# honglu2875/hironaka

Hardware: AMD Instinct MI355X
Metric: env-steps/sec at dim=3, max_pts=20, batch=65536; 1/2/4/8 GPUs (higher is better)
Workload: dtype f32

## Files before the change

hironaka_amd/csrc/hk_duo_kernel.h:

```cpp
#pragma once

#include "hk_fast_kernel.h"
#include "hk_lds_dma.h"

namespace hk {

constexpr int kDuoGames = kWave / 2;

#ifndef HK_DUO_LEGS
#define HK_DUO_LEGS 3
#endif
#ifdef HK_DUO_PROBE
constexpr int kDuoProbeRow = 48, kDuoProbeWaves = 4096;
static __device__ int32_t duo_probe_rows[kDuoProbeWaves * kDuoProbeRow];
#define HK_DUO_PROBE_PARAM , int32_t* probe = nullptr
#define HK_DUO_PROBE_ARG(p) , p
#else
#define HK_DUO_PROBE_PARAM
#define HK_DUO_PROBE_ARG(p)
#endif
constexpr bool kDuoLegDma = (HK_DUO_LEGS & 1) != 0, kDuoLegScan = (HK_DUO_LEGS & 2) != 0;

__device__ __forceinline__ int duo_other_i(int v) { return qperm_i<0xB1>(v); }
__device__ __forceinline__ float duo_other(float v) { return __int_as_float(duo_other_i(__float_as_int(v))); }

__device__ __forceinline__ uint64_t duo_ballot(bool p) { return __builtin_amdgcn_ballot_w64(p); }

template <int M, int D>
struct DuoGeom {
  using G = FastGeom<M, D>;
  static constexpr int CH = (G::C + 1) / 2;
  static constexpr int QH = (kDuoGames * G::Q + kWave - 1) / kWave;
  static constexpr bool kLean = CH * D <= 30;
};

template <int M, int D>
struct DuoSlabRegs {
  typename VecOf<FastGeom<M, D>::W>::type v[DuoGeom<M, D>::QH];
};

template <int M, int D, bool CONTIG>
__device__ __forceinline__ void duo_slab_issue_impl(DuoSlabRegs<M, D>& r, const float* base, int64_t in_stride,
                                                    int ngames, int lane) {
  using G = FastGeom<M, D>;
  using V = typename VecOf<G::W>::type;
  const int total = ngames * G::Q;
#pragma unroll
  for (int it = 0; it < DuoGeom<M, D>::QH; ++it) {
    int q = lane + it * kWave;
    q = q < total ? q : total - 1;
    r.v[it] = *reinterpret_cast<const V*>(base + slab_chunk_global<M, D, CONTIG>(q, in_stride));
  }
}

template <int M, int D>
__device__ __forceinline__ void duo_slab_issue(DuoSlabRegs<M, D>& r, const float* in, int64_t in_stride, int64_t g0,
                                               int ngames, int lane) {
  const float* base = in + g0 * in_stride;
  if (in_stride == FastGeom<M, D>::N) duo_slab_issue_impl<M, D, true>(r, base, in_stride, ngames, lane);
  else duo_slab_issue_impl<M, D, false>(r, base, in_stride, ngames, lane);
}

template <int M, int D>
__device__ __forceinline__ void duo_slab_commit(DuoSlabRegs<M, D>& r, float* lds, int ngames, int lane) {
  using G = FastGeom<M, D>;
  using V = typename VecOf<G::W>::type;
  const int total = ngames * G::Q;
#pragma unroll
  for (int it = 0; it < DuoGeom<M, D>::QH; ++it) asm volatile("" : "+v"(r.v[it]));
#pragma unroll
  for (int it = 0; it < DuoGeom<M, D>::QH; ++it) {
    const int q = lane + it * kWave;
    if (q < total) *reinterpret_cast<V*>(lds + slab_chunk_lds<M, D>(q)) = r.v[it];
  }
}

template <int M, int D>
struct DuoDma {
  using G = FastGeom<M, D>;
  static constexpr bool kShape = kDuoLegDma && G::W == 4 && G::S == G::N;
};

template <int M, int D>
__device__ __forceinline__ void duo_slab_dma(const float* base, float* image, int ngames, int lane) {
  using G = FastGeom<M, D>;
  constexpr int FULL = kDuoGames * G::Q;
  constexpr int QH = DuoGeom<M, D>::QH;
  constexpr int kImm = kDmaImm;
  static_assert(DuoDma<M, D>::kShape, "the image is the slab");
  const float* src = base + (unsigned)lane * 4;
  const unsigned total = (unsigned)ngames * G::Q;
  if (ngames == kDuoGames) {
    unrolled_while<0, QH>([&](auto ic) {
      constexpr int it = decltype(ic)::value;
      if ((it + 1) * kWave <= FULL || lane < FULL - it * kWave)
        lds_dma<16, (it * kWave * 16) % kImm>(src + (it * kWave * 16) / kImm * (kImm / 4),
                                             image + (it * kWave * 16) / kImm * (kImm / 4));
      return true;
    });
  } else {
    unrolled_while<0, QH>([&](auto ic) {
      constexpr int it = decltype(ic)::value;
      if ((unsigned)lane + it * kWave < total)
        lds_dma<16, (it * kWave * 16) % kImm>(src + (it * kWave * 16) / kImm * (kImm / 4),
                                             image + (it * kWave * 16) / kImm * (kImm / 4));
      return true;
    });
  }
}

constexpr int kStorePlain = 0, kStoreNT = 1, kStoreWT = 2;

template <int M, int D, bool CONTIG, int kBatch, int ST = kStorePlain>
__device__ __forceinline__ void duo_store_slab_impl(const float* lds, float* base, int64_t out_stride, int ngames,
                                                    int lane HK_DUO_PROBE_PARAM) {
  using G = FastGeom<M, D>;
  using V = typename VecOf<G::W>::type;
  constexpr int QH = DuoGeom<M, D>::QH;
  constexpr bool kWT = ST == kStoreWT && CONTIG && G::W == 4;
  const int total = ngames * G::Q;
#pragma unroll
  for (int i0 = 0; i0 < QH; i0 += kBatch) {
    V v[kBatch];
#pragma unroll
    for (int u = 0; u < kBatch; ++u) {
      int q = lane + (i0 + u) * kWave;
      q = q < kDuoGames * G::Q ? q : kDuoGames * G::Q - 1;
      v[u] = *reinterpret_cast<const V*>(lds + slab_chunk_lds<M, D>(q));
    }
#pragma unroll
    for (int u = 0; u < kBatch; ++u) asm volatile("" : "+v"(v[u]));
#ifdef HK_DUO_PROBE
    if (probe && lane == 0) probe[0] = (int32_t)wall_clock64();
#endif
    if constexpr (kWT) {
      typedef unsigned int vu4 __attribute__((ext_vector_type(4)));
      const uint64_t b = (uint64_t)base;
      const uint32_t blo = __builtin_amdgcn_readfirstlane((uint32_t)b), bhi = __builtin_amdgcn_readfirstlane((uint32_t)(b >> 32));
      const int bytes = __builtin_amdgcn_readfirstlane(total * G::W * (int)sizeof(float));
      const auto rsrc = __builtin_amdgcn_make_buffer_rsrc((void*)(((uint64_t)bhi << 32) | blo), 0, bytes, 0x00020000);
#pragma unroll
      for (int u = 0; u < kBatch; ++u) {
        const int q = lane + (i0 + u) * kWave;
        if (i0 + u < QH && q < total)
          __builtin_amdgcn_raw_buffer_store_b128(__builtin_bit_cast(vu4, v[u]), rsrc, q * G::W * (int)sizeof(float), 0,
                                                 16);
      }
    } else {
#pragma unroll
      for (int u = 0; u < kBatch; ++u) {
        const int q = lane + (i0 + u) * kWave;
        if (i0 + u < QH && q < total) {
          V* dst = reinterpret_cast<V*>(base + slab_chunk_global<M, D, CONTIG>(q, out_stride));
          if constexpr (ST != kStorePlain) __builtin_nontemporal_store(v[u], dst);
          else *dst = v[u];
        }
      }
    }
  }
}

template <int M, int D, int kBatch = DuoGeom<M, D>::QH, int ST = kStorePlain>
__device__ inline void duo_store_slab(const float* lds, float* out, int64_t out_stride, int64_t g0, int ngames,
                                      int lane HK_DUO_PROBE_PARAM) {
  float* base = out + g0 * out_stride;
  if (out_stride == FastGeom<M, D>::N) duo_store_slab_impl<M, D, true, kBatch, ST>(lds, base, out_stride, ngames, lane HK_DUO_PROBE_ARG(probe));
  else duo_store_slab_impl<M, D, false, kBatch, ST>(lds, base, out_stride, ngames, lane HK_DUO_PROBE_ARG(probe));
#ifdef HK_DUO_PROBE
  if (probe && lane == 0) probe[1] = (int32_t)wall_clock64();
#endif
}

struct DuoLadder {
  static constexpr int next_bucket(int nb) { return nb < 6 ? nb + 1 : nb + 2; }
};

template <int M, int CH, int D, int SB = CH>
__device__ __forceinline__ void duo_gather_slots(float (&q)[CH * D], const float* mine, uint32_t mask, int smax, int h) {
  mask = h ? (mask & (mask - 1)) : mask;
  unrolled_while<0, SB>([&](auto sc) {
    constexpr int s = decltype(sc)::value;
    if (s >= smax) return false;
    const bool has = mask != 0;
    const float* row = mine + (has ? mask_first(mask) : 0) * D;
    mask &= mask - 1;
    mask &= mask - 1;
#pragma unroll
    for (int k = 0; k < D; ++k) {
      const float v = row[k];
      q[s * D + k] = has ? v : INFINITY;
    }
    return true;
  });
}

template <int CH, int D, int NB, int SB = NB>
__device__ __forceinline__ void duo_gather_level(float (&q)[CH * D], const float* mine, const float* hole, uint32_t mask,
                                                 int h) {
  mask = h ? (mask & (mask - 1)) : mask;
  const float* row[NB];
#pragma unroll
  for (int s = 0; s < NB; ++s) {
    row[s] = mask != 0 ? mine + mask_first(mask) * D : hole;
    mask &= mask - 1;
    mask &= mask - 1;
  }
#pragma unroll
  for (int s = 0; s < NB; ++s)
#pragma unroll
    for (int k = 0; k < D; ++k) q[s * D + k] = row[s][k];
#pragma unroll
  for (int e = NB * D; e < SB * D; ++e) q[e] = INFINITY;
}

template <int M, int CH, int D, bool LEVELS, int SB = CH>
__device__ __forceinline__ void duo_gather(float (&q)[CH * D], const float* mine, const float* hole, uint32_t mask,
                                           int smax, int h) {
  if constexpr (LEVELS) {
    StagesFor<DuoLadder, SB>::run(smax, [&](auto nb) {
      duo_gather_level<CH, D, decltype(nb)::value, SB>(q, mine, hole, mask, h);
      return 0;
    });
  } else {
    duo_gather_slots<M, CH, D, SB>(q, mine, mask, smax, h);
  }
}

template <int CH, int D, int NB>
__device__ __forceinline__ uint32_t duo_scatter_level(const float (&q)[CH * D], float* mine, uint32_t mask, int h) {
  mask = h ? (mask & (mask - 1)) : mask;
  uint32_t alive = 0;
#pragma unroll
  for (int s = 0; s < NB; ++s) {
    if (mask != 0 && q[s * D] < INFINITY) {
      const int slot = mask_first(mask);
      alive |= 1u << slot;
      float* row = mine + slot * D;
#pragma unroll
      for (int k = 0; k < D; ++k) row[k] = q[s * D + k];
    }
    mask &= mask - 1;
    mask &= mask - 1;
  }
  return alive;
}

template <int M, int CH, int D, int SB = CH>
__device__ __forceinline__ uint32_t duo_scatter(const float (&q)[CH * D], float* mine, uint32_t mask, int smax, int h) {
  mask = h ? (mask & (mask - 1)) : mask;
  uint32_t alive = 0;
  unrolled_while<0, SB>([&](auto sc) {
    constexpr int s = decltype(sc)::value;
    if (s >= smax) return false;
    if (mask != 0 && q[s * D] < INFINITY) {
      const int slot = mask_first(mask);
      alive |= 1u << slot;
      float* row = mine + slot * D;
#pragma unroll
      for (int k = 0; k < D; ++k) row[k] = q[s * D + k];
    }
    mask &= mask - 1;
    mask &= mask - 1;
    return true;
  });
  return lanes_or<2>(alive);
}

template <int D>
__device__ __forceinline__ void duo_pad_rows(float* mine, uint32_t dead, float pad, int h) {
  dead = h ? (dead & (dead - 1)) : dead;
  while (dead != 0) {
    float* row = mine + mask_first(dead) * D;
#pragma unroll
    for (int k = 0; k < D; ++k) row[k] = pad;
    dead &= dead - 1;
    dead &= dead - 1;
  }
}

template <int M, int D>
__device__ __forceinline__ void duo_scan_half(const float* mine, float fill, int h, uint32_t& live, bool& ok) {
  static_assert(M <= 32, "the game's mask is one word");
  constexpr int C = (M + 1) / 2;
  const int i0 = h * C;
  const float* base = mine + i0 * D;
  uint32_t mask = 0;
  const uint32_t fill_bits = __float_as_uint(fill);
  uint32_t off = 0;
  bool okb = true;
#pragma unroll
  for (int r = 0; r < C; ++r) {
    const bool valid = (M % 2 == 0) || r + 1 < C || h == 0;
    uint32_t hi = __float_as_uint(base[r * D]), lo = hi;
#pragma unroll
    for (int k = 1; k < D; ++k) {
      const uint32_t u = __float_as_uint(base[r * D + k]);
      hi = u > hi ? u : hi;
      lo = u < lo ? u : lo;
    }
    const bool ge = hi < 0x7F800000u;
    if constexpr (DuoGeom<M, D>::kLean && kDuoLegScan) {
      const uint32_t differs = (hi ^ fill_bits) | (lo ^ fill_bits);
      off |= (ge || !valid) ? 0u : differs;
    } else {
      const bool fl = (lo == fill_bits) && (hi == fill_bits);
      okb &= (ge | fl | !valid);
    }
    mask |= (ge && valid) ? (1u << r) : 0u;
  }
  ok = (DuoGeom<M, D>::kLean && kDuoLegScan) ? off == 0u : okb;
  mask <<= i0;
  live = lanes_or<2>(mask);
}

template <bool DPP>
__device__ __forceinline__ int duo_wave_max(int v, int hi) {
  if constexpr (!DPP) return wave_max(v, hi);
  auto mx = [](int a, int b) { return a > b ? a : b; };
  v = mx(v, __builtin_amdgcn_update_dpp(0, v, 0x111, 0xF, 0xF, true));
  v = mx(v, __builtin_amdgcn_update_dpp(0, v, 0x112, 0xF, 0xF, true));
  v = mx(v, __builtin_amdgcn_update_dpp(0, v, 0x114, 0xF, 0xF, true));
  v = mx(v, __builtin_amdgcn_update_dpp(0, v, 0x118, 0xF, 0xF, true));
  v = mx(v, __builtin_amdgcn_update_dpp(0, v, 0x142, 0xA, 0xF, false));
  v = mx(v, __builtin_amdgcn_update_dpp(0, v, 0x143, 0xC, 0xF, false));
  return __builtin_amdgcn_readlane(v, kWave - 1);
}

template <int CH, int D, int NB>
__device__ __forceinline__ void d_newton(float (&q)[CH * D], int h) {
  float acc[NB], oth[NB];
#pragma unroll
  for (int i = 0; i + 1 < NB; ++i) {
#pragma unroll
    for (int j = i + 1; j < NB; ++j) {
      float t, u;
      diff_extrema<D>(&q[i * D], &q[j * D], t, u);
      const float vi = (t > 0.0f) ? -u : 1.0f;
      acc[j] = (i == 0) ? t : hk_fmin(acc[j], t);
      acc[i] = (i == 0 && j == 1) ? vi : hk_fmin(acc[i], vi);
    }
    __builtin_amdgcn_sched_barrier(0);
  }
  const bool late = h != 0;
#pragma unroll
  for (int b = 0; b < NB; ++b) {
    float o[D];
#pragma unroll
    for (int k = 0; k < D; ++k) o[k] = duo_other(q[b * D + k]);
    {
      float t, u;
      diff_extrema<D>(&q[b * D], o, t, u);
      const float va = (t > 0.0f || late) ? -u : 1.0f;
      acc[b] = (NB == 1) ? va : hk_fmin(acc[b], va);
      oth[b] = (u < 0.0f || !late) ? t : 1.0f;
    }
#pragma unroll
    for (int a = 0; a < b; ++a) {
      float t, u;
      diff_extrema<D>(&q[a * D], o, t, u);
      oth[b] = hk_fmin(oth[b], t);
      acc[a] = hk_fmin(acc[a], (t > 0.0f) ? -u : 1.0f);
    }
    __builtin_amdgcn_sched_barrier(0);
  }
#pragma unroll
  for (int r = 0; r < NB; ++r) {
    const bool r0 = acc[r] <= 0.0f, r1 = duo_other(oth[r]) <= 0.0f;
    const bool removed = r0 || r1;
#pragma unroll
    for (int k = 0; k < D; ++k) q[r * D + k] = removed ? INFINITY : q[r * D + k];
  }
}

template <int CH, int D, int NB>
__device__ __forceinline__ void d_shift_words(float (&q)[CH * D], uint32_t cmask, int axis, int np, unsigned flags) {
  bool apply = true;
  if (flags & HK_FLAG_AXIS_NOOP_IF_INVALID) apply = axis >= 0 && ((cmask >> axis) & 1u);
  if ((flags & HK_FLAG_IGNORE_ENDED) && np < 2) apply = false;
  const uint32_t onehot = apply ? 1u << (axis & 31) : 0u;
  uint32_t isax[D], in[D];
#pragma unroll
  for (int k = 0; k < D; ++k) {
    isax[k] = (uint32_t)((int32_t)(onehot << (31 - k)) >> 31);
    in[k] = (uint32_t)((int32_t)(cmask << (31 - k)) >> 31);
    asm volatile("" : "+v"(isax[k]), "+v"(in[k]));
  }
#pragma unroll
  for (int r = 0; r < NB; ++r) {
    float s = __uint_as_float(__float_as_uint(q[r * D]) & in[0]);
#pragma unroll
    for (int k = 1; k < D; ++k) s = s + __uint_as_float(__float_as_uint(q[r * D + k]) & in[k]);
#pragma unroll
    for (int k = 0; k < D; ++k)
      q[r * D + k] = __uint_as_float((__float_as_uint(s) & isax[k]) | (__float_as_uint(q[r * D + k]) & ~isax[k]));
  }
}

template <int CH, int D, int NB, bool BIN = false, bool WORDS = false>
__device__ __forceinline__ int d_stages(float (&q)[CH * D], const float (&c)[D], int axis, int np, int h,
                                        unsigned flags, unsigned stages, uint32_t cmask = 0) {
  static_assert(!WORDS || BIN, "the subset as bits");
  if (stages & HK_STAGE_SHIFT) {
    if constexpr (WORDS) d_shift_words<CH, D, NB>(q, cmask, axis, np, flags);
    else if constexpr (BIN) b_shift_mask<CH, D, NB>(q, cmask, axis, np, flags);
    else b_shift<CH, D, NB>(q, c, axis, np, flags);
  }
  if (stages & HK_STAGE_REPOSITION) reposition<2, CH, D, NB, BIN>(q, flags);
  if (stages & HK_STAGE_NEWTON) d_newton<CH, D, NB>(q, h);
  if (stages & HK_STAGE_RESCALE) rescale<2, CH, D, NB>(q, flags);
  return live_rows<2, CH, D, NB>(q);
}

template <int CH, int D, int NB, bool BIN = false>
struct DuoStagesFor {
  static constexpr int kNext = DuoLadder::next_bucket(NB);
  static __device__ __forceinline__ int run(float (&q)[CH * D], int smax, const float (&c)[D], int axis, int np,
                                            int h, unsigned flags, unsigned stages, uint32_t cmask = 0) {
    if constexpr (NB >= CH) {
      return d_stages<CH, D, CH, BIN>(q, c, axis, np, h, flags, stages, cmask);
    } else {
      if (smax <= NB) return d_stages<CH, D, NB, BIN>(q, c, axis, np, h, flags, stages, cmask);
      return DuoStagesFor<CH, D, kNext, BIN>::run(q, smax, c, axis, np, h, flags, stages, cmask);
    }
  }
};

template <int CH, int D>
__device__ __forceinline__ void duo_ranks_first(const float (&q)[CH * D], int smax, int (&rank)[CH]) {
#pragma unroll
  for (int s = 0; s < CH; ++s) rank[s] = 0;
  unrolled_while<0, CH>([&](auto bc) {
    constexpr int b = decltype(bc)::value;
    if (b >= smax) return false;
    float o[D];
#pragma unroll
    for (int k = 0; k < D; ++k) o[k] = duo_other(q[b * D + k]);
    const bool live_o = o[0] < INFINITY, live_b = q[b * D] < INFINITY;
    unrolled_while<0, CH>([&](auto ac) {
      constexpr int a = decltype(ac)::value;
      if (a >= smax) return false;
      rank[a] += (live_o && key_gt<D, kKeyFirst>(o, &q[a * D])) ? 1 : 0;
      if (a != b) rank[a] += (live_b && key_gt<D, kKeyFirst>(&q[b * D], &q[a * D])) ? 1 : 0;
      return true;
    });
    return true;
  });
}

template <int CH, int D>
__device__ __forceinline__ void duo_scatter_ranked(const float (&q)[CH * D], float* mine, const int (&rank)[CH], int smax) {
  unrolled_while<0, CH>([&](auto sc) {
    constexpr int s = decltype(sc)::value;
    if (s >= smax) return false;
    if (q[s * D] < INFINITY) {
      float* row = mine + rank[s] * D;
#pragma unroll
      for (int k = 0; k < D; ++k) row[k] = q[s * D + k];
    }
    return true;
  });
}

struct DuoPolicyCache {
  U4 r;
  uint32_t pair = 0xFFFFFFFFu;
};

__device__ inline void duo_policy_words(uint64_t gg, uint32_t step, uint64_t seed, DuoPolicyCache& cache, int h,
                                        uint32_t& host_word, uint32_t& agent_word) {
  const uint32_t block = step >> 2, pair = block >> 1;
  if (cache.pair != pair) {
    cache.r = philox4x32((uint32_t)gg, (uint32_t)(gg >> 32), (pair << 1) | (uint32_t)h, kStreamPolicy, seed);
    cache.pair = pair;
  }
  const uint32_t mine = u4_word(cache.r, step & 3u);
  const bool own = (int)(block & 1u) == h;
  uint32_t theirs = (uint32_t)duo_other_i((int)mine);
  asm volatile("" : "+v"(theirs));
  const uint32_t w = own ? mine : theirs;
  host_word = w & 0xFFFF0000u;
  agent_word = w << 16;
}

constexpr int kDuoZeilDpp = 6;

template <int CH, int D, int NB>
__device__ __forceinline__ int duo_zeillinger(const float (&q)[CH * D], int h, float* mine, int smax) {
  constexpr bool KEEP = NB <= kDuoZeilDpp;
  ZeilBest<D> best;
#pragma unroll
  for (int k = 0; k < D; ++k) best.bd[k] = 0.0f;
  if constexpr (KEEP) {
    float p[NB * D];
#pragma unroll
    for (int e = 0; e < NB * D; ++e) p[e] = duo_other(q[e]);
#pragma unroll
    for (int a = 0; a < NB; ++a) {
#pragma unroll
      for (int b = a + 1; b < NB; ++b)
        zeil_pair_cmp<D, true, false>(best, &q[a * D], &q[b * D], true, (128 * a + 2 * b) + 65 * h);
#pragma unroll
      for (int b = a; b < NB; ++b)
        zeil_pair_cmp<D, true>(best, &q[a * D], &p[b * D], (b > a) | (h == 0), (128 * a + 2 * b + 1) + 63 * h);
      if constexpr (NB > 3) __builtin_amdgcn_sched_barrier(0);
    }
  } else {
    __syncthreads();
#pragma unroll
    for (int s = 0; s < NB; ++s)
#pragma unroll
      for (int k = 0; k < D; ++k) mine[(2 * s + h) * D + k] = q[s * D + k];
    __syncthreads();
    const int n = 2 * smax;
    ZeilBest<D> second;
#pragma nounroll
    for (int i = h; i + 1 < n; i += 2) {
      float pi[D];
#pragma unroll
      for (int k = 0; k < D; ++k) pi[k] = mine[i * D + k];
#pragma nounroll
      for (int j = i + 1; j < n; j += 2) {
        float pj[D], pk[D];
        const int j2 = (j + 1 < n) ? j + 1 : j;
#pragma unroll
        for (int k = 0; k < D; ++k) {
          pj[k] = mine[j * D + k];
          pk[k] = mine[j2 * D + k];
        }
        zeil_pair2<D>(best, second, pi, pj, 64 * i + j, pi, pk, 64 * i + j + 1);
      }
    }
    zeil_merge<D, false>(best, second);
  }
  {
    ZeilBest<D> o;
    o.hi = (uint32_t)duo_other_i((int)best.hi);
    o.lo = (uint32_t)duo_other_i((int)best.lo);
    if constexpr (KEEP) {
#pragma unroll
      for (int k = 0; k < D; ++k) o.bd[k] = duo_other(best.bd[k]);
    }
    zeil_merge<D, KEEP>(best, o);
  }
  const bool have = best.have();
  if constexpr (!KEEP) {
    const int i = have ? (int)((best.lo & 0xFFFFu) >> 6) : 0, j = have ? (int)(best.lo & 63u) : 0;
#pragma unroll
    for (int k = 0; k < D; ++k) best.bd[k] = mine[i * D + k] - mine[j * D + k];
    __syncthreads();
  }
  int lo = 0, hi = 0;
  float vlo = best.bd[0], vhi = best.bd[0];
#pragma unroll
  for (int k = 1; k < D; ++k) {
    if (best.bd[k] < vlo) { vlo = best.bd[k]; lo = k; }
    if (best.bd[k] > vhi) { vhi = best.bd[k]; hi = k; }
  }
  if (!have || lo == hi) return 0;
  return encode_mask((1u << lo) | (1u << hi));
}

constexpr int kDuoPreBlocks = 6;

template <int D>
__device__ __forceinline__ void duo_policy_fill(uint8_t* act, uint64_t gg, uint32_t wb0, int nb, uint64_t seed,
                                                int host_policy, int agent_policy, int gi, int h) {
  static_assert(D <= 5 && D <= kPolicyShortDim, "an action travels as a byte; four steps per Philox block");
  auto put = [&](const U4& r, int b) {
    int cls, axis;
    uint32_t mask;
#pragma unroll
    for (int k = 0; k < 4; ++k) {
      const uint32_t w = u4_word(r, k);
      policy_from_words<D>(w & 0xFFFF0000u, w << 16, host_policy, agent_policy, cls, axis, mask, 0);
      act[(4 * b + k) * kDuoGames + gi] = (uint8_t)(mask | ((uint32_t)axis << 5));
    }
  };
#pragma nounroll
  for (int i = 0; i < kDuoPreBlocks; i += 4) {
    if (i >= nb) break;
    const int b0 = i + h, b1 = b0 + 2;
    if (i + 2 < nb) {
      const U4 r0 = philox4x32((uint32_t)gg, (uint32_t)(gg >> 32), wb0 + (uint32_t)b0, kStreamPolicy, seed);
      const U4 r1 = philox4x32((uint32_t)gg, (uint32_t)(gg >> 32), wb0 + (uint32_t)b1, kStreamPolicy, seed);
      put(r0, b0);
      if (b1 < kDuoPreBlocks) put(r1, b1);
    } else {
      const U4 r0 = philox4x32((uint32_t)gg, (uint32_t)(gg >> 32), wb0 + (uint32_t)b0, kStreamPolicy, seed);
      if (b0 < kDuoPreBlocks) put(r0, b0);
    }
  }
}

template <int M, int D, int MODE, int HOT = kHotNone, bool ACTS = false, bool ZEIL = false>
__global__ __launch_bounds__(kWave, 2) void duo_kernel(const float* in0, int64_t in_stride0, int batch0,
                                                       const Params prm) {
  static_assert(!ACTS || MODE == kModeRollout, "the small records ride on the plain rollout");
  static_assert(!ZEIL || (MODE == kModeRollout && HOT == kHotNone && !ACTS), "Zeillinger's host: plain rollouts");
  constexpr bool kRec = MODE == kModeRolloutRec;
  constexpr bool kRoll = MODE == kModeRollout || kRec;
  constexpr bool kPartialPublish = MODE == kModeRollout && !ZEIL && DuoGeom<M, D>::kLean;
  constexpr bool kLevelDeal = MODE == kModeRollout && DuoGeom<M, D>::kLean;
  using G = FastGeom<M, D>;
  constexpr int CH = DuoGeom<M, D>::CH;
  static_assert(M <= 32, "the live mask of a game travels as 32 bits");
  __shared__ __align__(16) float lds[kDuoGames * G::S];
  __shared__ float cbuf[kDuoGames * D];
  __shared__ float hole_row[D];
  __shared__ __align__(16) uint8_t pol[(MODE == kModeRollout) ? (4 * kDuoPreBlocks + 1) * kDuoGames : 16];
  const int lane = threadIdx.x;
  const int h = lane & 1, gi = lane >> 1;
  const int64_t g0 = (int64_t)blockIdx.x * kDuoGames;
  const int64_t left = (int64_t)batch0 - g0;
  const int ngames = (int)(left < kDuoGames ? left : kDuoGames);
  const bool active = gi < ngames;
  const bool leader = active && h == 0;
  const int64_t g = g0 + gi;
#ifdef HK_DUO_PROBE
  __shared__ int32_t probe_buf[32];
  if (lane < 32) probe_buf[lane] = 0;
  const long long probe_t0 = wall_clock64();
  long long probe_t1 = 0, probe_t2 = 0;
  int probe_steps = 0, probe_smax = 0;
#endif
  const bool has_ids = kRoll && prm.game_ids != nullptr;
  uint32_t raw_id = 0;
  DuoSlabRegs<M, D> slab;
  uint64_t gg;
  bool dma = false;
  if constexpr (DuoDma<M, D>::kShape) {
    if (has_ids) {
      if (active) raw_id = (uint32_t)prm.game_ids[g];
      __builtin_amdgcn_sched_barrier(0);
      duo_slab_issue<M, D>(slab, in0, in_stride0, g0, ngames, lane);
      __builtin_amdgcn_sched_barrier(0);
      asm volatile("" : "+v"(raw_id));
      gg = prm.game_offset + (uint64_t)raw_id;
    } else {
      dma = in_stride0 == G::N && ((uintptr_t)in0 & 15u) == 0;
      if (dma) duo_slab_dma<M, D>(in0 + g0 * G::N, lds, ngames, lane);
      else duo_slab_issue<M, D>(slab, in0, in_stride0, g0, ngames, lane);
      __builtin_amdgcn_sched_barrier(0);
      gg = prm.game_offset + (uint64_t)g;
    }
  } else {
    if (has_ids && active) raw_id = (uint32_t)prm.game_ids[g];
    __builtin_amdgcn_sched_barrier(0);
    duo_slab_issue<M, D>(slab, in0, in_stride0, g0, ngames, lane);
    __builtin_amdgcn_sched_barrier(0);
    gg = prm.game_offset + (has_ids ? (uint64_t)raw_id : (uint64_t)g);
  }
  uint32_t pol_b0 = prm.step_offset >> 2;
  const uint32_t pol_last = (prm.steps > 0) ? (prm.step_offset + (uint32_t)prm.steps - 1u) >> 2 : pol_b0;
  if constexpr (MODE == kModeRollout && !ZEIL) {
    const uint32_t nb = pol_last - pol_b0 + 1u;
    duo_policy_fill<D>(pol, gg, pol_b0, (int)(nb < (uint32_t)kDuoPreBlocks ? nb : (uint32_t)kDuoPreBlocks), prm.seed,
                       HOT ? (int)HK_HOST_RANDOM : prm.host_policy,
                       (HOT == kHotJax) ? (int)HK_AGENT_RANDOM
                                        : (HOT == kHotTorch) ? (int)HK_AGENT_RANDOM_LEGAL : prm.agent_policy, gi, h);
  }
#ifdef HK_DUO_PROBE
  if (lane == 0) probe_buf[21] = (int32_t)wall_clock64();
#endif
  float* mine = lds + gi * G::S;
  const float pad = (float)prm.pad;
  const unsigned flags = (HOT == kHotJax) ? (unsigned)HK_SEM_JAX : (HOT == kHotTorch) ? kHotTorchFlags : prm.flags;
  const unsigned stages = HOT ? (unsigned)(HK_STAGE_SHIFT | HK_STAGE_REPOSITION | HK_STAGE_NEWTON) : prm.stages;
  const float fill = ((flags & HK_SEM_MASK) == HK_SEM_JAX) ? -1.0f : pad;
  const int nsteps = kRoll ? prm.steps : 1;
  constexpr bool kEndSort = MODE == kModeRollout && HOT == kHotNone;
  const bool end_sort = kEndSort && nsteps > 0 && (stages & HK_STAGE_NEWTON) &&
                        ((flags & HK_SEM_MASK) == HK_SEM_LIST || (flags & HK_FLAG_COMPACT_SORTED));
  bool rescale_pending = false;
  PolicyCache pcache;
  DuoPolicyCache dcache;
  float c[D];
  int axis_in = -1;
#pragma unroll
  for (int k = 0; k < D; ++k) c[k] = 0.0f;
  RawActions<D> raw;
  const bool fetch_actions = !kRoll && (stages & HK_STAGE_SHIFT) && active;
  if (fetch_actions) fast_fetch_actions<D>(prm, g, M, raw);
  if constexpr (DuoDma<M, D>::kShape) {
    if (dma) wait_vmem_all();
    else duo_slab_commit<M, D>(slab, lds, ngames, lane);
  } else {
    duo_slab_commit<M, D>(slab, lds, ngames, lane);
  }
  if (kLevelDeal && lane < D) hole_row[lane] = INFINITY;
  if (fetch_actions) fast_decode_actions<D>(prm, raw, c, axis_in);
  __syncthreads();
#ifdef HK_DUO_PROBE
  if (lane == 0) probe_buf[22] = (int32_t)wall_clock64();
#endif

  uint32_t gmask;
  bool ok;
  duo_scan_half<M, D>(mine, fill, h, gmask, ok);
  if (!active) {
    gmask = 0;
    ok = true;
  }
  int np = mask_pop(gmask);
#ifdef HK_DUO_PROBE
  asm volatile("" : "+v"(np));
  if (lane == 0) probe_buf[24] = (int32_t)wall_clock64();
#endif
  int nmax = duo_wave_max<DuoGeom<M, D>::kLean && kDuoLegScan>(np, M);
  const bool exact = (fill == pad) && __all(ok) && nmax <= G::C;

  if (!exact) {
    float* cs = cbuf + gi * D;
    np = leader ? num_points<float>(mine, M, D) : 2;
    int length = (np < 2) ? 0 : -1;
    if (kRoll && prm.count_ws) {
      const unsigned long long b0 = __ballot(leader && np < 2);
      if (lane == 0) count_add(prm.count_ws + blockIdx.x, (uint32_t)__popcll(b0));
    }
    for (int t = 0; t < nsteps; ++t) {
      int axis = axis_in, cls = 0;
      if (kRec && prm.obs_out) {
        __syncthreads();
        duo_store_slab<M, D, 2>(lds, (float*)prm.obs_out + (int64_t)t * prm.batch * G::N, (int64_t)G::N, g0, ngames, lane);
        __syncthreads();
      }
      if (kRoll) {
        uint32_t mask;
        const int zc = (prm.host_policy == HK_HOST_ZEILLINGER && leader) ? zeillinger_game<float>(mine, prm.m, prm.d) : 0;
        fast_policy<D>(prm, gg, prm.step_offset + (uint32_t)t, pcache, cls, axis, mask, zc);
        if (leader)
          for (int k = 0; k < prm.d; ++k) cs[k] = (float)((mask >> k) & 1u);
      } else if ((stages & HK_STAGE_SHIFT) && leader) {
        load_coords<float>(prm, g, cs);
      }
      const bool prev_done = np < 2;
      if (leader) {
        stages_game<float>(mine, prm.m, prm.d, cs, axis, pad, stages, flags);
        np = num_points<float>(mine, prm.m, prm.d);
      }
      const bool done = np < 2;
      if (done && length < 0) length = t + 1;
      if (kRoll && prm.count_ws) {
        const unsigned long long bd = __ballot(leader && done);
        if (lane == 0) count_add(prm.count_ws + (size_t)(t + 1) * prm.count_stride + blockIdx.x, (uint32_t)__popcll(bd));
      }
      if ((kRec || ACTS) && leader) {
        const int64_t at = (int64_t)t * prm.batch + g;
        if (prm.r_host_class_out) prm.r_host_class_out[at] = cls;
        if (prm.r_axis_out) prm.r_axis_out[at] = axis;
        if (prm.r_done_out) prm.r_done_out[at] = done;
        if (prm.r_reward_out) prm.r_reward_out[at] = prm.reward_sign * (float)(done && !prev_done);
      }
      if (!kRoll && leader) {
        if (prm.done_out) prm.done_out[g] = done;
        if (prm.prev_done_out) prm.prev_done_out[g] = prev_done;
        if (prm.reward_out) prm.reward_out[g] = prm.reward_sign * (float)(done && !prev_done);
        if (prm.num_points_out) prm.num_points_out[g] = np;
      }
    }
    if (kRoll && leader && prm.game_length_out) prm.game_length_out[g] = length;
    __syncthreads();
    duo_store_slab<M, D>(lds, (float*)prm.out, prm.out_stride, g0, ngames, lane);
    return;
  }

  if (kPartialPublish && h == 0) reinterpret_cast<uint32_t*>(cbuf)[gi] = gmask;
  int smax = (nmax + 1) >> 1;
#ifdef HK_DUO_PROBE
  probe_t1 = wall_clock64();
  probe_smax = smax;
#endif
  float q[CH * D];
  if constexpr (!kLevelDeal) {
#pragma unroll
    for (int e = 0; e < CH * D; ++e) q[e] = INFINITY;
  }
  duo_gather<M, CH, D, kLevelDeal>(q, mine, hole_row, gmask, smax, h);
#ifdef HK_DUO_PROBE
  {
    float sink = 0.0f;
#pragma unroll
    for (int e = 0; e < CH * D; ++e) sink += (q[e] < INFINITY) ? q[e] : 0.0f;
    asm volatile("" : "+v"(sink));
    if (lane == 0) probe_buf[23] = (int32_t)wall_clock64();
  }
#endif
  if (!active) np = 2;
  int length = (np < 2) ? 0 : -1;
  if (kRoll && prm.count_ws) {
    const unsigned long long b0 = __ballot(leader && np < 2);
    if (lane == 0) count_add(prm.count_ws + blockIdx.x, (uint32_t)__popcll(b0));
  }
  uint32_t* count_slot = (kRoll && prm.count_ws) ? prm.count_ws + blockIdx.x : nullptr;
  uint32_t count_stride = prm.count_stride;
  uint32_t step0 = prm.step_offset;
  uint64_t seed = prm.seed;
  int host_policy = HOT ? (int)HK_HOST_RANDOM : prm.host_policy;
  int agent_policy = (HOT == kHotJax) ? (int)HK_AGENT_RANDOM
                                      : (HOT == kHotTorch) ? (int)HK_AGENT_RANDOM_LEGAL : prm.agent_policy;
  if (HOT)
    asm volatile("" : "+s"(count_slot), "+s"(count_stride), "+s"(step0), "+s"(seed));
  else
    asm volatile("" : "+s"(count_slot), "+s"(count_stride), "+s"(step0), "+s"(seed), "+s"(host_policy),
                 "+s"(agent_policy));
  static_assert(kDuoGames == 32 && kWave == 64, "flush_records: two steps of the wave's games per instruction");
  int32_t* rec_cls = ACTS ? prm.r_host_class_out : nullptr;
  int32_t* rec_axis = ACTS ? prm.r_axis_out : nullptr;
  uint8_t* rec_done = ACTS ? prm.r_done_out : nullptr;
  float* rec_reward = ACTS ? prm.r_reward_out : nullptr;
  int64_t rec_batch = prm.batch;
  float rec_sign = prm.reward_sign;
  if constexpr (ACTS)
    asm volatile("" : "+s"(rec_cls), "+s"(rec_axis), "+s"(rec_done), "+s"(rec_reward), "+s"(rec_batch), "+s"(rec_sign));
  constexpr bool want_small = ACTS;
  int t_rec = 0;
  auto flush_records = [&](int t_end) {
    if (t_rec < t_end) {
      const int gsel = lane & (kDuoGames - 1), sub = lane >> 5;
      const int lg = __shfl(length, gsel * 2);
      const bool gok = gsel < ngames;
      const int64_t off = (int64_t)sub * rec_batch + gsel;
      const uint8_t* w = pol + (int)(step0 + (uint32_t)t_rec - (pol_b0 << 2)) * kDuoGames + lane;
      for (int ta = t_rec; ta < t_end; ta += 2, w += 2 * kDuoGames) {
        const int tt = ta + sub;
        if (gok && tt < t_end) {
          const uint32_t a = *w;
          const int64_t row = (int64_t)ta * rec_batch + g0;
          if (rec_cls) (rec_cls + row)[off] = encode_mask(a & 31u);
          if (rec_axis) (rec_axis + row)[off] = (int32_t)(a >> 5);
          if (rec_done) (rec_done + row)[off] = lg >= 0 && tt + 1 >= lg;
          if (rec_reward) (rec_reward + row)[off] = rec_sign * (float)(lg >= 1 && tt + 1 == lg);
        }
      }
    }
    t_rec = t_end;
  };
  if constexpr (MODE == kModeRollout) {
    static_assert(CH <= 6 || CH % 2 == 0, "bucket ladder: 1..6, then even numbers");
    uint64_t amask = duo_ballot(active), lmask = duo_ballot(leader);
    asm volatile("" : "+s"(amask), "+s"(lmask));
    int open_steps = (np < 2) ? -1 : 0;
    auto length_at = [&](int tt) { return open_steps == tt ? -1 : open_steps + 1; };
    int t = 0;
    bool stop = false;
    while (t < nsteps && !stop) {
    if (!ZEIL && (uint32_t)((step0 + (uint32_t)t) >> 2) - pol_b0 >= (uint32_t)kDuoPreBlocks) {
      if constexpr (want_small) {
        length = length_at(t);
        flush_records(__builtin_amdgcn_readfirstlane(t));
      }
      __syncthreads();
      pol_b0 = (step0 + (uint32_t)t) >> 2;
      const uint32_t nb = pol_last - pol_b0 + 1u;
      duo_policy_fill<D>(pol, gg, pol_b0, (int)(nb < (uint32_t)kDuoPreBlocks ? nb : (uint32_t)kDuoPreBlocks), seed,
                         host_policy, agent_policy, gi, h);
      __syncthreads();
    }
    const uint32_t wend_abs = (pol_b0 + (uint32_t)kDuoPreBlocks) << 2;
    const int tw = (!ZEIL && wend_abs - step0 < (uint32_t)nsteps) ? (int)(wend_abs - step0) : nsteps;
    uint32_t a_next = ZEIL ? 0u : pol[(int)(step0 + (uint32_t)t - (pol_b0 << 2)) * kDuoGames + gi];
    Levels<DuoLadder, CH>::run([&](auto nbc, auto loc) {
      constexpr int NB = decltype(nbc)::value, LO = decltype(loc)::value;
      if (!((smax > LO || LO == 0) && t < tw && !stop)) return;
#ifndef HK_NO_SETPRIO
      if (t >= 10) __builtin_amdgcn_s_setprio(3);
      else if constexpr (NB >= 6) __builtin_amdgcn_s_setprio(3);
      else if constexpr (NB >= 4) __builtin_amdgcn_s_setprio(2);
      else if constexpr (NB >= 2) __builtin_amdgcn_s_setprio(1);
      else __builtin_amdgcn_s_setprio(0);
#endif
      auto play = [&](int tend) {
        while (t < tend) {
          uint32_t mask;
          int axis;
          if constexpr (ZEIL) {
            static_assert(NB <= kDuoZeilDpp || 2 * NB <= M, "the rolled pair loop parks ranks 0 .. 2 NB - 1 in the game's M rows");
            const int zc = (duo_ballot(np >= 2) & amask) != 0 ? duo_zeillinger<CH, D, NB>(q, h, mine, smax) : 0;
            uint32_t ra, rb;
            int cls;
            duo_policy_words(gg, step0 + (uint32_t)t, seed, dcache, h, ra, rb);
            policy_from_words<D>(ra, rb, host_policy, agent_policy, cls, axis, mask, zc);
          } else {
            const uint32_t a = a_next;
            a_next = pol[(int)(step0 + (uint32_t)t + 1u - (pol_b0 << 2)) * kDuoGames + gi];
            mask = a & 31u;
            axis = (int)(a >> 5);
          }
          const unsigned st = (end_sort && t + 1 == nsteps) ? (stages & ~(unsigned)HK_STAGE_RESCALE) : stages;
          rescale_pending = end_sort && t + 1 == nsteps && (stages & HK_STAGE_RESCALE);
          const int np_new = d_stages<CH, D, NB, true, (NB == 1)>(q, c, axis, np, h, flags, st, mask);
#ifdef HK_DUO_PROBE
          if (lane == 0 && t == 0) probe_buf[20] = (int32_t)wall_clock64();
#endif
          if constexpr (NB == 1) {
            const uint64_t live = duo_ballot(q[0] < INFINITY);
            const uint64_t open = live & (live >> 1) & lmask;
            open_steps += __builtin_amdgcn_inverse_ballot_w64(open) ? 1 : 0;
            np = __builtin_amdgcn_inverse_ballot_w64(open | (open << 1)) ? 2 : 0;
            if (open == 0) {
              uint32_t any_bits = __float_as_uint(q[0]);
#pragma unroll
              for (int k = 1; k < D; ++k) any_bits |= __float_as_uint(q[k]);
              if ((duo_ballot(any_bits != 0u) & live & amask) == 0) {
                stop = true;
                tend = 0;
              }
            }
          } else {
            np = np_new;
            open_steps += (leader && np >= 2) ? 1 : 0;
            if ((duo_ballot(np >= 2 * smax - 1) & amask) == 0) {
              int left = nsteps - 1 - t;
              asm volatile("" : "+s"(left));
              if (left > 0) {
                __syncthreads();
                if constexpr (kLevelDeal) {
                  gmask = lanes_or<2>(duo_scatter_level<CH, D, NB>(q, mine, gmask, h));
                  __syncthreads();
                  nmax = duo_wave_max<DuoGeom<M, D>::kLean && kDuoLegScan>(active ? np : 0, 2 * smax - 2);
                  smax = (nmax + 1) >> 1;
                  duo_gather_level<CH, D, NB>(q, mine, hole_row, gmask, h);
                } else {
                  gmask = duo_scatter<M, CH, D, NB>(q, mine, gmask, smax, h);
                  __syncthreads();
                  const int sprev = smax;
                  nmax = duo_wave_max<DuoGeom<M, D>::kLean && kDuoLegScan>(active ? np : 0, 2 * smax - 2);
                  smax = (nmax + 1) >> 1;
                  duo_gather_slots<M, CH, D, NB>(q, mine, gmask, sprev, h);
                }
                tend = smax <= LO ? 0 : tend;
              }
            }
          }
#ifdef HK_DUO_PROBE
          if (lane == 0 && t < 24) probe_buf[t] = (int32_t)((((uint32_t)wall_clock64()) << 4) | (uint32_t)(smax & 15));
#endif
          ++t;
        }
      };
      if constexpr (NB == 1) {
        play(tw < 10 ? tw : 10);
        if (t < tw && !stop) {
#ifndef HK_NO_SETPRIO
          __builtin_amdgcn_s_setprio(3);
#endif
          play(tw);
        }
      } else {
        play(tw);
      }
    });
    }
    length = length_at(t);
#ifdef HK_DUO_PROBE
    probe_steps = t;
    probe_t2 = wall_clock64();
#endif
    if (count_slot) add_length_counts(count_slot, count_stride, 1, nsteps, leader, length, lane);
    if constexpr (want_small) {
      for (;;) {
        const uint32_t wend = ((pol_b0 + (uint32_t)kDuoPreBlocks) << 2) - step0;
        const int te = __builtin_amdgcn_readfirstlane((wend < (uint32_t)nsteps) ? (int)wend : nsteps);
        flush_records(te);
        if (te >= nsteps) break;
        __syncthreads();
        pol_b0 = (step0 + (uint32_t)te) >> 2;
        const uint32_t nb = pol_last - pol_b0 + 1u;
        duo_policy_fill<D>(pol, gg, pol_b0, (int)(nb < (uint32_t)kDuoPreBlocks ? nb : (uint32_t)kDuoPreBlocks), seed,
                           host_policy, agent_policy, gi, h);
        __syncthreads();
      }
    }
  }
  const bool want_obs = kRec && prm.obs_out != nullptr;
  const bool want_records = kRec && (prm.r_host_class_out || prm.r_axis_out || prm.r_done_out || prm.r_reward_out);
  for (int t = 0; MODE != kModeRollout && t < nsteps; ++t) {
    int axis = axis_in, cls = 0;
    if (want_obs) {
      __syncthreads();
      if (h == 0) fill_image<M, D>(mine, pad);
      __syncthreads();
      duo_scatter<M, CH, D>(q, mine, gmask, smax, h);
      __syncthreads();
      duo_store_slab<M, D, 2>(lds, (float*)prm.obs_out + (int64_t)t * prm.batch * G::N, (int64_t)G::N, g0, ngames, lane);
    }
    uint32_t mask = 0;
    if (kRoll) {
      uint32_t ra, rb;
      duo_policy_words(gg, step0 + (uint32_t)t, seed, dcache, h, ra, rb);
      policy_from_words<D>(ra, rb, host_policy, agent_policy, cls, axis, mask, 0);
    }
    const bool prev_done = np < 2;
    const unsigned st = (end_sort && t + 1 == nsteps) ? (stages & ~(unsigned)HK_STAGE_RESCALE) : stages;
    rescale_pending = end_sort && t + 1 == nsteps && (stages & HK_STAGE_RESCALE);
    np = DuoStagesFor<CH, D, 1, kRoll>::run(q, smax, c, axis, np, h, flags, st, mask);
    if (!active) np = 2;
    const bool done = np < 2;
    if (done && length < 0) length = t + 1;
    if (!kRoll && leader) {
      if (prm.done_out) prm.done_out[g] = done;
      if (prm.prev_done_out) prm.prev_done_out[g] = prev_done;
      if (prm.reward_out) prm.reward_out[g] = prm.reward_sign * (float)(done && !prev_done);
      if (prm.num_points_out) prm.num_points_out[g] = np;
    }
    if (want_records && leader) {
      const int64_t at = (int64_t)t * prm.batch + g;
      if (prm.r_host_class_out) prm.r_host_class_out[at] = cls;
      if (prm.r_axis_out) prm.r_axis_out[at] = axis;
      if (prm.r_done_out) prm.r_done_out[at] = done;
      if (prm.r_reward_out) prm.r_reward_out[at] = prm.reward_sign * (float)(done && !prev_done);
    }
    const unsigned long long bd = __ballot(leader && done);
    if (count_slot && lane == 0) count_add(count_slot + (size_t)(t + 1) * count_stride, (uint32_t)__popcll(bd));
    if (MODE == kModeRollout && smax == 1 && bd == __ballot(leader) && t + 1 < nsteps) {
      bool still = true;
#pragma unroll
      for (int k = 0; k < D; ++k) still &= (q[k] == 0.0f);
      still |= !(q[0] < INFINITY);
      if (!__any(active && !still)) {
        if (count_slot && lane == 0)
          for (int tt = t + 1; tt < nsteps; ++tt) count_add(count_slot + (size_t)(tt + 1) * count_stride, (uint32_t)__popcll(bd));
        break;
      }
    }
    if (t + 1 < nsteps && !__any(active && ((np + 1) >> 1) >= smax)) {
      __syncthreads();
      gmask = duo_scatter<M, CH, D>(q, mine, gmask, smax, h);
      __syncthreads();
      const int sprev = smax;
      nmax = duo_wave_max<DuoGeom<M, D>::kLean && kDuoLegScan>(active ? np : 0, 2 * smax - 2);
      smax = (nmax + 1) >> 1;
      duo_gather_slots<M, CH, D>(q, mine, gmask, sprev, h);
    }
  }
  if (kRoll && leader && prm.game_length_out) prm.game_length_out[g] = length;
#ifdef HK_DUO_PROBE
  if (lane == 0) probe_buf[25] = (int32_t)wall_clock64();
#endif

  __syncthreads();
  if (kPartialPublish && !end_sort) {
    const uint32_t alive = duo_scatter<M, CH, D>(q, mine, gmask, smax, h);
    duo_pad_rows<D>(mine, reinterpret_cast<const uint32_t*>(cbuf)[gi] & ~alive, pad, h);
  } else {
    if (h == 0) fill_image<M, D>(mine, pad);
    __syncthreads();
    if (kEndSort && end_sort) {
      int rank[CH];
      duo_ranks_first<CH, D>(q, smax, rank);
      if (rescale_pending) rescale<2, CH, D, CH>(q, flags);
      duo_scatter_ranked<CH, D>(q, mine, rank, smax);
    } else {
      duo_scatter<M, CH, D>(q, mine, gmask, smax, h);
    }
  }
  __syncthreads();
#ifdef HK_DUO_PROBE
  if (lane == 0) probe_buf[26] = (int32_t)wall_clock64();
#endif
  constexpr int kFinalStore = MODE != kModeRollout ? kStorePlain : DuoGeom<M, D>::kLean ? kStoreWT : kStoreNT;
  duo_store_slab<M, D, DuoGeom<M, D>::QH, kFinalStore>(lds, (float*)prm.out, prm.out_stride, g0, ngames,
                                                       lane HK_DUO_PROBE_ARG(probe_buf + 27));
#ifdef HK_DUO_PROBE
  if (kRoll && lane == 0 && blockIdx.x < (unsigned)kDuoProbeWaves) {
    int32_t* w = duo_probe_rows + blockIdx.x * kDuoProbeRow;
    w[0] = (int32_t)probe_t0;
    w[1] = (int32_t)probe_t1;
    w[2] = (int32_t)probe_t2;
    w[3] = (int32_t)wall_clock64();
    w[4] = probe_steps;
    w[5] = probe_smax;
    w[6] = (int32_t)blockIdx.x;
    w[7] = (int32_t)__builtin_amdgcn_s_getreg((4 << 0) | (0 << 6) | (31 << 11));
    for (int i = 0; i < 32; ++i) w[8 + i] = probe_buf[i];
  }
#endif
}

inline int device_simds() {
  static int cached[16] = {0};
  int dev = 0;
  if (hipGetDevice(&dev) != hipSuccess || dev < 0 || dev >= 16) dev = 0;
  if (!cached[dev]) {
    int cus = 0;
    if (hipDeviceGetAttribute(&cus, hipDeviceAttributeMultiprocessorCount, dev) != hipSuccess || cus <= 0) cus = 256;
    (void)hipGetLastError();
    cached[dev] = 4 * cus;
  }
  return cached[dev];
}

inline bool duo_supported(const Params& prm, int dtype) {
  if ((prm.mode != kModeRollout && prm.mode != kModeStep) || prm.m > 32) return false;
  if (prm.mode == kModeStep && (prm.class_out || (prm.stages & kStageFeatureSorts))) return false;
  if (prm.mode == kModeRollout && prm.host_policy == HK_HOST_ZEILLINGER && any_records(prm)) return false;
  if (sorted_output(prm) && (prm.mode != kModeRollout || any_records(prm))) return false;
  return fast_supported(prm, dtype);
}

template <int M, int D>
int launch_duo_t(Params prm, hipStream_t stream) {
  const unsigned grid = (unsigned)(((int64_t)prm.batch + kDuoGames - 1) / kDuoGames);
  prm.games_per_block = kDuoGames;
  launch_prepare();
  const bool records = prm.obs_out != nullptr;
  const bool acts = small_records_only(prm);
  const int hot = (prm.mode == kModeRollout && !records) ? fast_hot_config(prm) : kHotNone;
  if (prm.mode == kModeRollout && records)
    hipLaunchKernelGGL((duo_kernel<M, D, kModeRolloutRec>), dim3(grid), dim3(kWave), 0, stream, (const float*)prm.in,
                       prm.in_stride, prm.batch, prm);
  else if (prm.mode == kModeRollout && prm.host_policy == HK_HOST_ZEILLINGER)
    hipLaunchKernelGGL((duo_kernel<M, D, kModeRollout, kHotNone, false, true>), dim3(grid), dim3(kWave), 0, stream,
                       (const float*)prm.in, prm.in_stride, prm.batch, prm);
  else if (prm.mode == kModeRollout && acts && hot == kHotJax)
    hipLaunchKernelGGL((duo_kernel<M, D, kModeRollout, kHotJax, true>), dim3(grid), dim3(kWave), 0, stream,
                       (const float*)prm.in, prm.in_stride, prm.batch, prm);
  else if (prm.mode == kModeRollout && acts)
    hipLaunchKernelGGL((duo_kernel<M, D, kModeRollout, kHotNone, true>), dim3(grid), dim3(kWave), 0, stream,
                       (const float*)prm.in, prm.in_stride, prm.batch, prm);
  else if (prm.mode == kModeStep && prm.flags == HK_SEM_JAX &&
           prm.stages == (HK_STAGE_SHIFT | HK_STAGE_REPOSITION | HK_STAGE_NEWTON))
    hipLaunchKernelGGL((duo_kernel<M, D, kModeStep, kHotJax>), dim3(grid), dim3(kWave), 0, stream,
                       (const float*)prm.in, prm.in_stride, prm.batch, prm);
  else if (prm.mode == kModeStep)
    hipLaunchKernelGGL((duo_kernel<M, D, kModeStep>), dim3(grid), dim3(kWave), 0, stream, (const float*)prm.in,
                       prm.in_stride, prm.batch, prm);
  else if (hot == kHotJax)
    hipLaunchKernelGGL((duo_kernel<M, D, kModeRollout, kHotJax>), dim3(grid), dim3(kWave), 0, stream,
                       (const float*)prm.in, prm.in_stride, prm.batch, prm);
  else if (hot == kHotTorch)
    hipLaunchKernelGGL((duo_kernel<M, D, kModeRollout, kHotTorch>), dim3(grid), dim3(kWave), 0, stream,
                       (const float*)prm.in, prm.in_stride, prm.batch, prm);
  else
    hipLaunchKernelGGL((duo_kernel<M, D, kModeRollout>), dim3(grid), dim3(kWave), 0, stream, (const float*)prm.in,
                       prm.in_stride, prm.batch, prm);
  return launch_status();
}

#ifndef HK_SPEC_TU
#define HK_X(M_, D_) extern template int launch_duo_t<M_, D_>(Params, hipStream_t);
HK_FAST_SPECS(HK_X)
#undef HK_X

inline int launch_duo(const Params& prm, hipStream_t stream) {
#define HK_X(M_, D_) if (prm.m == M_ && prm.d == D_) return launch_duo_t<M_, D_>(prm, stream);
  HK_FAST_SPECS(HK_X)
#undef HK_X
  return HK_ERR_UNSUPPORTED;
}
#endif

}
```

Before: 64.87 billion.

## Tally episode lengths via LDS histogram and widen policy Philox fill to three chains

When the step count fits in a wave, each block now builds a per-length histogram in LDS with workgroup-scoped atomics, sums it with DPP, and issues one global count_add per occupied length. This replaces the existing add_length_counts path and the separate ballot for already-finished games. It also lets duo_policy_fill generate three independent Philox blocks per iteration instead of two, to expose more instruction-level parallelism. The cost is an extra __syncthreads and LDS buffer, plus higher register pressure from the third Philox chain.

Measured after the change: 67.65 billion (median of 6 runs). 4.3% higher.

```diff
diff --git a/hironaka_amd/csrc/hk_duo_kernel.h b/hironaka_amd/csrc/hk_duo_kernel.h
--- a/hironaka_amd/csrc/hk_duo_kernel.h
+++ b/hironaka_amd/csrc/hk_duo_kernel.h
@@ -8,7 +8,7 @@
 constexpr int kDuoGames = kWave / 2;
 
 #ifndef HK_DUO_LEGS
-#define HK_DUO_LEGS 3
+#define HK_DUO_LEGS 7
 #endif
 #ifdef HK_DUO_PROBE
 constexpr int kDuoProbeRow = 48, kDuoProbeWaves = 4096;
@@ -20,6 +20,7 @@
 #define HK_DUO_PROBE_ARG(p)
 #endif
 constexpr bool kDuoLegDma = (HK_DUO_LEGS & 1) != 0, kDuoLegScan = (HK_DUO_LEGS & 2) != 0;
+constexpr bool kDuoLegCounts = (HK_DUO_LEGS & 4) != 0;
 
 __device__ __forceinline__ int duo_other_i(int v) { return qperm_i<0xB1>(v); }
 __device__ __forceinline__ float duo_other(float v) { return __int_as_float(duo_other_i(__float_as_int(v))); }
@@ -326,6 +327,21 @@
   return __builtin_amdgcn_readlane(v, kWave - 1);
 }
 
+__device__ __forceinline__ void duo_length_counts(uint32_t* hist, uint32_t* slot, uint32_t stride, int nsteps, bool counted,
+                                                  int length, int lane) {
+  hist[lane] = 0u;
+  if (counted && length >= 0) __hip_atomic_fetch_add(hist + length, 1u, __ATOMIC_RELAXED, __HIP_MEMORY_SCOPE_WORKGROUP);
+  __syncthreads();
+  uint32_t v = hist[lane];
+  v += (uint32_t)__builtin_amdgcn_update_dpp(0, (int)v, 0x111, 0xF, 0xF, true);
+  v += (uint32_t)__builtin_amdgcn_update_dpp(0, (int)v, 0x112, 0xF, 0xF, true);
+  v += (uint32_t)__builtin_amdgcn_update_dpp(0, (int)v, 0x114, 0xF, 0xF, true);
+  v += (uint32_t)__builtin_amdgcn_update_dpp(0, (int)v, 0x118, 0xF, 0xF, true);
+  v += (uint32_t)__builtin_amdgcn_update_dpp(0, (int)v, 0x142, 0xA, 0xF, false);
+  v += (uint32_t)__builtin_amdgcn_update_dpp(0, (int)v, 0x143, 0xC, 0xF, false);
+  if (lane <= nsteps && v) count_add(slot + (size_t)lane * stride, v);
+}
+
 template <int CH, int D, int NB>
 __device__ __forceinline__ void d_newton(float (&q)[CH * D], int h) {
   float acc[NB], oth[NB];
@@ -560,9 +576,18 @@
   return encode_mask((1u << lo) | (1u << hi));
 }
 
-constexpr int kDuoPreBlocks = 6;
-
-template <int D>
+#ifndef HK_DUO_PRE_BLOCKS
+#define HK_DUO_PRE_BLOCKS 6
+#endif
+#ifndef HK_DUO_FILL_CHAINS
+#define HK_DUO_FILL_CHAINS 3
+#endif
+constexpr int kDuoPreBlocks = HK_DUO_PRE_BLOCKS;
+constexpr int kDuoFillChains = HK_DUO_FILL_CHAINS;
+static_assert(kDuoPreBlocks >= 2 && kDuoPreBlocks % 2 == 0, "a pair of lanes fills two blocks at a time");
+static_assert(kDuoFillChains == 2 || kDuoFillChains == 3, "two or three chains per lane");
+
+template <int D, int CHAINS = 2>
 __device__ __forceinline__ void duo_policy_fill(uint8_t* act, uint64_t gg, uint32_t wb0, int nb, uint64_t seed,
                                                 int host_policy, int agent_policy, int gi, int h) {
   static_assert(D <= 5 && D <= kPolicyShortDim, "an action travels as a byte; four steps per Philox block");
@@ -577,10 +602,18 @@
     }
   };
 #pragma nounroll
-  for (int i = 0; i < kDuoPreBlocks; i += 4) {
+  for (int i = 0; i < kDuoPreBlocks; i += 2 * CHAINS) {
     if (i >= nb) break;
     const int b0 = i + h, b1 = b0 + 2;
-    if (i + 2 < nb) {
+    if (CHAINS == 3 && i + 4 < nb) {
+      const int b2 = b0 + 4;
+      const U4 r0 = philox4x32((uint32_t)gg, (uint32_t)(gg >> 32), wb0 + (uint32_t)b0, kStreamPolicy, seed);
+      const U4 r1 = philox4x32((uint32_t)gg, (uint32_t)(gg >> 32), wb0 + (uint32_t)b1, kStreamPolicy, seed);
+      const U4 r2 = philox4x32((uint32_t)gg, (uint32_t)(gg >> 32), wb0 + (uint32_t)b2, kStreamPolicy, seed);
+      put(r0, b0);
+      put(r1, b1);
+      if (b2 < kDuoPreBlocks) put(r2, b2);
+    } else if (i + 2 < nb) {
       const U4 r0 = philox4x32((uint32_t)gg, (uint32_t)(gg >> 32), wb0 + (uint32_t)b0, kStreamPolicy, seed);
       const U4 r1 = philox4x32((uint32_t)gg, (uint32_t)(gg >> 32), wb0 + (uint32_t)b1, kStreamPolicy, seed);
       put(r0, b0);
@@ -608,6 +641,8 @@
   __shared__ float cbuf[kDuoGames * D];
   __shared__ float hole_row[D];
   __shared__ __align__(16) uint8_t pol[(MODE == kModeRollout) ? (4 * kDuoPreBlocks + 1) * kDuoGames : 16];
+  constexpr bool kHistCounts = MODE == kModeRollout && kDuoLegCounts;
+  __shared__ uint32_t hist[kHistCounts ? kWave : 1];
   const int lane = threadIdx.x;
   const int h = lane & 1, gi = lane >> 1;
   const int64_t g0 = (int64_t)blockIdx.x * kDuoGames;
@@ -654,7 +689,7 @@
   const uint32_t pol_last = (prm.steps > 0) ? (prm.step_offset + (uint32_t)prm.steps - 1u) >> 2 : pol_b0;
   if constexpr (MODE == kModeRollout && !ZEIL) {
     const uint32_t nb = pol_last - pol_b0 + 1u;
-    duo_policy_fill<D>(pol, gg, pol_b0, (int)(nb < (uint32_t)kDuoPreBlocks ? nb : (uint32_t)kDuoPreBlocks), prm.seed,
+    duo_policy_fill<D, kDuoFillChains>(pol, gg, pol_b0, (int)(nb < (uint32_t)kDuoPreBlocks ? nb : (uint32_t)kDuoPreBlocks), prm.seed,
                        HOT ? (int)HK_HOST_RANDOM : prm.host_policy,
                        (HOT == kHotJax) ? (int)HK_AGENT_RANDOM
                                         : (HOT == kHotTorch) ? (int)HK_AGENT_RANDOM_LEGAL : prm.agent_policy, gi, h);
@@ -787,7 +822,8 @@
 #endif
   if (!active) np = 2;
   int length = (np < 2) ? 0 : -1;
-  if (kRoll && prm.count_ws) {
+  const bool hist_counts = kHistCounts && nsteps < kWave;
+  if (kRoll && prm.count_ws && !hist_counts) {
     const unsigned long long b0 = __ballot(leader && np < 2);
     if (lane == 0) count_add(prm.count_ws + blockIdx.x, (uint32_t)__popcll(b0));
   }
@@ -956,7 +992,13 @@
     probe_steps = t;
     probe_t2 = wall_clock64();
 #endif
-    if (count_slot) add_length_counts(count_slot, count_stride, 1, nsteps, leader, length, lane);
+    if (count_slot) {
+      if (hist_counts) duo_length_counts(hist, count_slot, count_stride, nsteps, leader, length, lane);
+      else add_length_counts(count_slot, count_stride, 1, nsteps, leader, length, lane);
+    }
+#ifdef HK_DUO_PROBE
+    if (lane == 0) probe_buf[29] = (int32_t)wall_clock64();
+#endif
     if constexpr (want_small) {
       for (;;) {
         const uint32_t wend = ((pol_b0 + (uint32_t)kDuoPreBlocks) << 2) - step0;
```
